# ingonyama-zk/icicle

Hardware: AMD Instinct MI355X
Metric: bn254_msm_2^26_per_sec (higher is better)
Workload: dtype u32x8 (254-bit integer field, 29-bit-limb Montgomery); 1 GPU; BN254 G1 MSM, 2^26 uniform scalars x 2^26 distinct affine bases per GPU, batch 1, inputs resident in HBM, precompute_factor 1

## Files before the change

icicle_amd/csrc/bigfield.hpp:

```cpp
#pragma once
#include <cstdint>
#include "field_consts.h"
#include "mont_asm.hpp"

#if defined(__HIPCC__)
  #include <hip/hip_runtime.h>
  #define HD __host__ __device__ __forceinline__
#else
  #define HD inline __attribute__((always_inline))
#endif

#ifdef BIGFIELD_BOUNDS
  #include <cassert>
  #include <cstdio>
  #define BF_BOUND_DECL                                                                                                \
    double bnd = 0;                                                                                                    \
    bool sg = false;                                                                                                   \
    double slo = 0, shi = 0, llo = 0, lhi = 0, tlo = 0, thi = 0;
  #define BF_SET_BOUND(x, v) ((x).bnd = (v), (x).sg = false)
  #define BF_ASSERT(cond, msg)                                                                                         \
    do {                                                                                                               \
      if (!(cond)) {                                                                                                   \
        fprintf(stderr, "bigfield bound violation: %s (%s:%d)\n", msg, __FILE__, __LINE__);                            \
        assert(false);                                                                                                 \
// ... 414 lines not shown
        r.l[i] = a.l[i] + b.l[i];
#ifdef BIGFIELD_BOUNDS
      const SB x = sview(a), y = sview(b);
      sset(r, SB{x.lo + y.lo, x.hi + y.hi, x.llo + y.llo, x.lhi + y.lhi, x.tlo + y.tlo, x.thi + y.thi});
#endif
      return r;
    }
    static HD fe ssub(const fe& a, const fe& b)
    {
      fe r;
#pragma unroll
      for (int i = 0; i < N; i++)
        r.l[i] = a.l[i] - b.l[i];
#ifdef BIGFIELD_BOUNDS
      const SB x = sview(a), y = sview(b);
      sset(r, SB{x.lo - y.hi, x.hi - y.lo, x.llo - y.lhi, x.lhi - y.llo, x.tlo - y.thi, x.thi - y.tlo});
#endif
      return r;
    }
    static HD fe sneg(const fe& a)
    {
      fe r;
#pragma unroll
      for (int i = 0; i < N; i++)
        r.l[i] = 0u - a.l[i];
#ifdef BIGFIELD_BOUNDS
      const SB x = sview(a);
      sset(r, SB{-x.hi, -x.lo, -x.lhi, -x.llo, -x.thi, -x.tlo});
#endif
      return r;
    }
    static HD fe sadd2(const fe& a, const fe& b)
    {
      fe r;
#pragma unroll
      for (int i = 0; i < N; i++)
        r.l[i] = (a.l[i] << 1) + b.l[i];
#ifdef BIGFIELD_BOUNDS
      const SB x = sview(a), y = sview(b);
      sset(r, SB{2 * x.lo + y.lo, 2 * x.hi + y.hi, 2 * x.llo + y.llo, 2 * x.lhi + y.lhi, 2 * x.tlo + y.tlo, 2 * x.thi + y.thi});
#endif
      return r;
    }
    static HD fe scneg(const fe& a, bool negate)
    {
      fe r;
      const uint32_t s = negate ? 0xffffffffu : 0u, o = negate ? 1u : 0u;
#pragma unroll
      for (int i = 0; i < N; i++)
        r.l[i] = (a.l[i] ^ s) + o;
#ifdef BIGFIELD_BOUNDS
      const SB x = sview(a);
      auto mn = [](double u, double v) { return u < v ? u : v; };
      auto mx = [](double u, double v) { return u > v ? u : v; };
      sset(r, SB{mn(x.lo, -x.hi), mx(x.hi, -x.lo), mn(x.llo, -x.lhi), mx(x.lhi, -x.llo), mn(x.tlo, -x.thi), mx(x.thi, -x.tlo)});
#endif
      return r;
    }
    static HD fe snormalise(const fe& a)
    {
      fe r;
      int32_t c = 0;
#pragma unroll
      for (int i = 0; i < N - 1; i++) {
        const int32_t t = (int32_t)a.l[i] + c;
        r.l[i] = (uint32_t)t & MASK;
        c = t >> RB;
      }
      r.l[N - 1] = a.l[N - 1] + (uint32_t)c;
#ifdef BIGFIELD_BOUNDS
      const SB x = sview(a);
      double clo = 0, chi = 0;
      for (int i = 0; i < N - 1; i++) {
        BF_ASSERT(x.llo + clo >= -I32_LIM && x.lhi + chi <= I32_LIM, "snormalise: limb + carry can leave int32");
        clo = __builtin_floor((x.llo + clo) / (double)(1u << RB));
        chi = __builtin_floor((x.lhi + chi) / (double)(1u << RB));
      }
      BF_ASSERT(x.tlo + clo >= -I32_LIM && x.thi + chi <= I32_LIM, "snormalise: top limb + carry can leave int32");
      sset(r, normalised(x.lo, x.hi));
#endif
      return r;
    }
    template <int K>
    static HD fe to_unsigned(const fe& a)
    {
      fe r;
      int32_t c = 0;
#pragma unroll
      for (int i = 0; i < N - 1; i++) {
        const int32_t t = (int32_t)(a.l[i] + kp<K>(i)) + c;
        r.l[i] = (uint32_t)t & MASK;
        c = t >> RB;
      }
      r.l[N - 1] = a.l[N - 1] + kp<K>(N - 1) + (uint32_t)c;
#ifdef BIGFIELD_BOUNDS
      const SB x = sview(a);
      BF_ASSERT(x.lo >= -(double)K, "to_unsigned: value can be below -K*p");
      BF_ASSERT(smag(x, 0) + (double)(1u << RB) + 8.0 <= I32_LIM && smag(x, N - 1) + (double)kp<K>(N - 1) + 8.0 <= I32_LIM, "to_unsigned: limb + K*p + carry can leave int32");
      BF_SET_BOUND(r, x.hi + (double)K);
      BF_ASSERT(r.bnd <= max_bound(), "to_unsigned result bound");
#endif
      return r;
    }

    template <bool TWO>
    static HD void sprod_generic(fe& r, const fe& a, const fe& b, const fe& c, const fe& d)
    {
      uint32_t m[N], o[N];
      int64_t acc = 0;
      auto term = [](uint32_t x, uint32_t y) { return (int64_t)(int32_t)x * (int64_t)(int32_t)y; };
#pragma unroll
      for (int k = 0; k < N; k++) {
#pragma unroll
        for (int i = 0; i <= k; i++) {
          acc += term(a.l[i], b.l[k - i]);
          if constexpr (TWO) acc += term(c.l[i], d.l[k - i]);
          if (i < k) acc += (int64_t)m[i] * (int64_t)PR::P[k - i];
        }
        m[k] = ((uint32_t)acc * PR::PINV) & MASK;
        acc += (int64_t)m[k] * (int64_t)PR::P[0];
        acc >>= RB;
      }
#pragma unroll
      for (int k = N; k < 2 * N - 1; k++) {
#pragma unroll
        for (int i = k - N + 1; i < N; i++) {
          acc += term(a.l[i], b.l[k - i]);
          if constexpr (TWO) acc += term(c.l[i], d.l[k - i]);
          acc += (int64_t)m[i] * (int64_t)PR::P[k - i];
        }
        o[k - N] = (uint32_t)acc & MASK;
        acc >>= RB;
      }
      o[N - 1] = (uint32_t)acc;
#pragma unroll
      for (int i = 0; i < N; i++)
        r.l[i] = o[i];
    }
    static HD fe smul(const fe& a, const fe& b)
    {
      fe r;
#ifdef BIGFIELD_BOUNDS
      sset_mul(r, a, b);
#endif
#if defined(__HIP_DEVICE_COMPILE__) && !defined(BIGFIELD_NO_ASM)
      if constexpr (N == 9) {
        mont_smul_asm9<PR>(r.l, a.l, b.l);
        return r;
      }
#endif
      sprod_generic<false>(r, a, b, a, b);
      return r;
    }
    static HD void smul_inplace(fe& a, const fe& b)
    {
#if defined(__HIP_DEVICE_COMPILE__) && !defined(BIGFIELD_NO_ASM)
      if constexpr (N == 9) {
        mont_smul_inplace_asm9<PR>(a.l, b.l);
        return;
      }
#endif
      a = smul(a, b);
    }
    static HD fe ssqr(const fe& a)
    {
      fe r;
// ... 197 lines not shown
```

icicle_amd/csrc/ec.hpp:

```cpp
#pragma once
#include "bigfield.hpp"
#include "fq2.hpp"
#include <type_traits>

#if defined(__HIPCC__)
  #define EC_NOINLINE __host__ __device__ __noinline__
#else
  #define EC_NOINLINE __attribute__((noinline))
#endif

namespace icicle_hip {

  template <class C>
  struct EC {
    using F = std::conditional_t<C::EXT_DEGREE == 2, Fq2Ops<typename C::fq>, FieldOps<typename C::fq>>;
    using fe = typename F::fe;
    static constexpr int N32 = F::N32;

    struct Aff {
      fe x, y;
    };
    struct XYZZ {
      fe x, y, zz, zzz;
    };
// ... 153 lines not shown
          return;
        }
      }
      fe PPP = F::smul(P, PP);
      fe Q = F::smul(acc.x, PP);
      fe t = F::sadd2(Q, PPP);
      fe X3 = F::snormalise(F::ssub(F::ssqr(R), t));
      fe d = F::ssub(Q, X3);
      acc.y = F::sneg(acc.y);
      F::smul_add_inplace_c(acc.y, R, d, PPP);
      F::smul_inplace(acc.zz, PP);
      F::smul_inplace(acc.zzz, PPP);
      acc.x = X3;
    }

    static HD Proj proj_identity()
    {
      Proj r;
      r.x = F::zero();
      r.y = F::one();
      r.z = F::zero();
      return r;
    }
    static HD Proj to_proj(const XYZZ& a, bool empty)
    {
      if (empty) return proj_identity();
      Proj r;
      if constexpr (SIGNED_MADD) {
        XYZZ s = a;
        F::sassume_normalised(s.x, -4.0, 6.0);
        F::sassume_normalised(s.y, -1.0, 4.0);
        F::sassume_normalised(s.zz, -0.25, 2.0);
        F::sassume_normalised(s.zzz, -0.25, 2.0);
        const fe zz1 = F::smul(s.zz, F::plain_one());
        r.x = F::template to_unsigned<1>(F::smul(s.x, s.zzz));
        r.y = F::template to_unsigned<1>(F::smul(s.y, s.zz));
        r.z = F::template to_unsigned<1>(F::smul(zz1, s.zzz));
      } else {
        const fe zz1 = F::mul_base(a.zz, F::base_plain_one());
        r.x = F::mul(a.x, a.zzz);
        r.y = F::mul(a.y, a.zz);
        r.z = F::mul(zz1, a.zzz);
      }
      return r;
    }
    static HD Proj to_proj(const Aff& a)
    {
      Proj r;
      r.x = a.x;
      r.y = a.y;
      r.z = F::one();
      return r;
    }
    static HD Proj add(const Proj& p, const Proj& q)
    {
      if constexpr (C::EXT_DEGREE == 2)
        return add_call(p, q);
      else
        return add_body(p, q);
    }
    static EC_NOINLINE Proj add_call(const Proj& p, const Proj& q) { return add_body(p, q); }
    static HD Proj add_body(const Proj& p, const Proj& q)
    {
      fe t0 = F::mul(p.x, q.x);
      fe t1 = F::mul(p.y, q.y);
      fe t2 = F::mul(p.z, q.z);
      fe t3 = F::mul(F::add(p.x, p.y), F::add(q.x, q.y));
      t3 = F::template sub<4>(t3, F::add(t0, t1));
      fe t4 = F::mul(F::add(p.y, p.z), F::add(q.y, q.z));
      t4 = F::template sub<4>(t4, F::add(t1, t2));
      fe t5 = F::mul(F::add(p.x, p.z), F::add(q.x, q.z));
      t5 = F::template sub<4>(t5, F::add(t0, t2));
      fe t0_3 = F::add(F::dbl(t0), t0);
      fe bt2 = F::mul(b3(), t2);
      fe z3 = F::add(t1, bt2);
      fe t1m = F::template sub<2>(t1, bt2);
      fe y3 = F::mul(b3(), t5);
      Proj r;
      r.x = F::template sub<2>(F::mul(t3, t1m), F::mul(t4, y3));
      r.y = F::add(F::mul(t1m, z3), F::mul(y3, t0_3));
      r.z = F::add(F::mul(z3, t4), F::mul(t0_3, t3));
      return r;
    }
    static HD Proj dbl(const Proj& p)
    {
      if constexpr (C::EXT_DEGREE == 2)
        return dbl_call(p);
      else
        return dbl_body(p);
    }
    static EC_NOINLINE Proj dbl_call(const Proj& p) { return dbl_body(p); }
    static HD Proj dbl_body(const Proj& p)
    {
      fe t0 = F::sqr(p.y);
      fe z8 = F::dbl(F::dbl(F::dbl(t0)));
      fe t1 = F::mul(p.y, p.z);
      fe t2 = F::mul(b3(), F::sqr(p.z));
      Proj r;
      fe x3 = F::mul(t2, z8);
      fe y3 = F::add(t0, t2);
      r.z = F::mul(t1, z8);
      fe t2_3 = F::add(F::dbl(t2), t2);
      fe t0m = F::template sub<4>(t0, t2_3);
      r.y = F::add(x3, F::mul(t0m, y3));
      r.x = F::dbl(F::mul(t0m, F::mul(p.x, p.y)));
      return r;
    }

    struct Jac {
      fe x, y, z;
    };
    static HD Jac to_jac(const Proj& p)
    {
      Jac r;
      fe zz = F::sqr(p.z);
      r.x = F::mul(p.x, p.z);
      r.y = F::mul(p.y, zz);
      r.z = p.z;
      return r;
    }
    static HD Proj from_jac(const Jac& j)
    {
      if (F::is_zero(j.z)) return proj_identity();
      Proj r;
      fe zz = F::sqr(j.z);
      r.x = F::mul(j.x, j.z);
      r.y = j.y;
      r.z = F::mul(zz, j.z);
      return r;
    }
    static HD Jac dbl_jac(const Jac& p)
    {
      fe A = F::sqr(p.x);
      fe B = F::sqr(p.y);
      fe CC = F::sqr(B);
      fe t = F::sqr(F::add(p.x, B));
      fe D = F::below4(F::dbl(F::template sub<4>(t, F::add(A, CC))));
      fe E = F::add(F::dbl(A), A);
      fe Fv = F::sqr(E);
      Jac r;
      r.x = F::below4(F::template sub<8>(Fv, F::dbl(D)));
      fe m = F::mul(E, F::template sub<4>(D, r.x));
      fe c8 = F::dbl(F::below4(F::dbl(F::dbl(CC))));
      r.y = F::below4(F::template sub<8>(m, c8));
      r.z = F::dbl(F::mul(p.y, p.z));
      return r;
    }

    static HD Jac dbl_jac_lazy(const Jac& p)
    {
      if constexpr (C::EXT_DEGREE == 2) {
        return dbl_jac(p);
      } else {
        fe A = F::sqr(p.x);
        fe B = F::sqr(p.y);
        fe CC = F::sqr(B);
        fe t = F::sqr(F::add(p.x, B));
        fe D = F::below4(F::dbl(F::template sub<4>(t, F::add(A, CC))));
        fe E = F::add(F::dbl(A), A);
        fe Fv = F::sqr(E);
        Jac r;
        r.x = F::template sub<8>(Fv, F::dbl(D));
        fe m = F::mul(E, F::template sub<16>(D, r.x));
        r.y = F::template sub<16>(m, F::dbl(F::dbl(F::dbl(CC))));
        r.z = F::dbl(F::mul(p.y, p.z));
        return r;
// ... 105 lines not shown
```

icicle_amd/csrc/msm_impl.hpp:

```cpp
#pragma once
#include "common.h"
#include "ec.hpp"
#include "ec_dbl_quad.hpp"
#include "msm_plan.h"
#include <algorithm>
#include <tuple>

namespace icicle_hip {

  template <class C>
  __global__ __launch_bounds__(256) void k_bases_stage(const uint32_t* __restrict__ in, uint32_t* __restrict__ out, size_t ncoord, bool in_refmont)
  {
    using BF = FieldOps<typename C::fq>;
    size_t t = blockIdx.x * (size_t)blockDim.x + threadIdx.x;
    if (t >= ncoord) return;
    uint32_t w[BF::N32];
#pragma unroll
    for (int i = 0; i < BF::N32; i++)
      w[i] = in[t * BF::N32 + i];
    if (in_refmont) {
      typename BF::fe cst;
#pragma unroll
      for (int k = 0; k < BF::N; k++)
        cst.l[k] = C::fq::REFMONT_TO_CANON[k];
// ... 733 lines not shown
    }
    const size_t wp = bucket / nb;
    bases += (wp / wpf) * bases_stride;
    const uint32_t total = count[bucket];
    const uint32_t cnt = min(total - min(total, start), seg);
    const uint32_t* src = sorted + wp * cap + offs[bucket] + start;
    typename E::XYZZ acc;
    bool empty = true;
    auto load4 = [&](uint32_t j) {
      uint4 v;
      __builtin_memcpy(&v, src + j, 16);
      return v;
    };
    uint4 cur = load4(0), nxt = cur;
    for (uint32_t j = 0; j < cnt; j++) {
      if ((j & 3u) == 0) nxt = load4(j + 4);
      const uint32_t e = cur.x;
      cur.x = cur.y, cur.y = cur.z, cur.z = cur.w;
      if ((j & 3u) == 3u) cur = nxt;
      const uint4* p = reinterpret_cast<const uint4*>(bases + (size_t)(e & 0x7fffffffu) * PW);
      uint32_t w[PW];
#pragma unroll
      for (int q = 0; q < PW / 4; q++) {
        const uint4 v = p[q];
        w[4 * q] = v.x;
        w[4 * q + 1] = v.y;
        w[4 * q + 2] = v.z;
        w[4 * q + 3] = v.w;
      }
      if (__builtin_expect(E::words_are_zero(w), 0)) continue;
      typename E::Aff a = E::cneg_madd(E::load_plain(w), (e >> 31) != 0);
      E::madd(acc, empty, a);
    }
    *dst = E::to_proj(acc, empty);
  }

  template <class C>
  __global__ __launch_bounds__(64) void k_fold_overflow(typename EC<C>::Proj* __restrict__ buckets, const typename EC<C>::Proj* __restrict__ ovf_part, const OvfSeg* __restrict__ ovf, const uint32_t* __restrict__ firsts, const uint32_t* __restrict__ ovf_count, uint32_t ovf_cap)
  {
    using E = EC<C>;
    __shared__ typename E::Proj sh[64];
    const uint32_t n = min(ovf_count[0], ovf_cap), nfirst = ovf_count[1];
    const uint32_t mx = ovf_count[2];
    const uint32_t G = mx <= 2 ? 1u : (mx <= 32 ? 4u : (mx <= 256 ? 16u : 64u)), per_block = 64 / G;
    const uint32_t lane = threadIdx.x, sub = lane / G, gl = lane % G;
    for (uint32_t q0 = blockIdx.x * per_block; q0 < nfirst; q0 += gridDim.x * per_block) {
      const uint32_t q = q0 + sub;
      const bool act = q < nfirst;
      const uint32_t o = act ? firsts[q] : 0;
      const uint32_t ne = act ? min(ovf[o].nextra, n - o) : 0;
      typename E::Proj v = E::proj_identity();
      for (uint32_t k = gl; k < ne; k += G)
        v = E::add(v, ovf_part[o + k]);
      sh[lane] = v;
      __syncthreads();
      for (uint32_t s = G / 2; s >= 1; s >>= 1) {
        if (gl < s) {
          v = E::add(v, sh[lane + s]);
          sh[lane] = v;
        }
        __syncthreads();
      }
      if (act && gl == 0) buckets[ovf[o].bucket] = E::add(buckets[ovf[o].bucket], v);
      __syncthreads();
    }
  }

  template <class C>
  struct ReduceWindowLanes {
    static constexpr int value = (sizeof(typename EC<C>::Proj) * 256 <= 60 * 1024) ? 256 : 128;
  };
  template <class P>
  __device__ __forceinline__ P proj_shfl_down(const P& v, int d)
  {
    static_assert(sizeof(P) % 4 == 0, "projective point is a whole number of words");
    P r;
    const uint32_t* src = reinterpret_cast<const uint32_t*>(&v);
    uint32_t* dst = reinterpret_cast<uint32_t*>(&r);
#pragma unroll
    for (size_t i = 0; i < sizeof(P) / 4; i++)
      dst[i] = __shfl_down(src[i], d);
    return r;
  }
  template <class C>
  __device__ __forceinline__ typename EC<C>::Proj wave_suffix_sum(typename EC<C>::Proj v, int lane)
  {
    using E = EC<C>;
    for (int d = 1; d < 64; d <<= 1) {
      const typename E::Proj o = proj_shfl_down(v, d);
      if (lane + d < 64) v = E::add(v, o);
    }
    return v;
  }
  template <class C>
  __device__ __forceinline__ typename EC<C>::Proj wave_sum(typename EC<C>::Proj v, int lane)
  {
    using E = EC<C>;
    for (int d = 32; d >= 1; d >>= 1) {
      const typename E::Proj o = proj_shfl_down(v, d);
      if (lane < d) v = E::add(v, o);
    }
    return v;
  }

  template <class C>
  __global__ __launch_bounds__(64) void k_reduce_wave(const typename EC<C>::Proj* __restrict__ buckets, typename EC<C>::Proj* __restrict__ chunkV, typename EC<C>::Proj* __restrict__ chunkT, typename EC<C>::Proj* __restrict__ winsum_direct, uint32_t nb_stride, uint32_t nb_wide, uint32_t m_wide, uint32_t seg_lo, uint32_t nsegr, uint32_t nlo_w, uint32_t nseg_lo, uint32_t m_lo)
  {
    using E = EC<C>;
    const int lane = threadIdx.x;
    const uint32_t nlo_blocks = nlo_w * nseg_lo;
    size_t wp;
    uint32_t ch, nb, lch;
    uint32_t m;
    if (blockIdx.x < nlo_blocks) {
      wp = blockIdx.x / nseg_lo, lch = blockIdx.x % nseg_lo, ch = lch, nb = nb_wide / 2, m = m_lo;
    } else {
      const uint32_t r = blockIdx.x - nlo_blocks;
      wp = nlo_w + r / nsegr, lch = r % nsegr, ch = seg_lo + lch, nb = nb_wide, m = m_wide;
    }
    const size_t oi = wp * nsegr + lch;
    const uint32_t k0 = ch * 64u * m;
    const typename E::Proj* b = buckets + wp * nb_stride;
    typename E::Proj line = E::proj_identity(), tri0 = E::proj_identity();
    for (int i = (int)m - 1; i >= 0; i--) {
      const uint32_t k = k0 + 64u * (uint32_t)i + (uint32_t)lane;
      tri0 = E::add(tri0, line);
      if (k < nb) line = E::add(line, b[k]);
    }
    const typename E::Proj suf = wave_suffix_sum<C>(line, lane);
    typename E::Proj x = proj_shfl_down(suf, 1);
    if (lane == 63) x = E::proj_identity();
    for (int q = 0; q < 6; q++)
      tri0 = E::dbl(tri0);
    const typename E::Proj v = wave_sum<C>(E::add(x, tri0), lane);
    if (lane == 0) {
      if (winsum_direct) {
        winsum_direct[oi] = E::add(v, suf);
      } else {
        chunkV[oi] = v;
        chunkT[oi] = suf;
      }
    }
  }

  template <class C>
  __global__ __launch_bounds__(64) void k_reduce_small(const typename EC<C>::Proj* __restrict__ buckets, typename EC<C>::Proj* __restrict__ winsum, uint32_t nb, uint32_t lw_log, uint32_t nwindows)
  {
    using E = EC<C>;
    const uint32_t lane = threadIdx.x, LW = 1u << lw_log, rows = nb >> lw_log;
    const uint32_t sl = lane & (LW - 1u);
    const size_t wp = (size_t)blockIdx.x * (64u >> lw_log) + (lane >> lw_log);
    const bool act = wp < nwindows;
    const typename E::Proj* b = buckets + (act ? wp : 0) * nb;
    typename E::Proj line = E::proj_identity(), tri0 = E::proj_identity();
    for (int i = (int)rows - 1; i >= 0; i--) {
      tri0 = E::add(tri0, line);
      if (act) line = E::add(line, b[(uint32_t)i * LW + sl]);
    }
    typename E::Proj suf = line;
    for (uint32_t d = 1; d < LW; d <<= 1) {
      const typename E::Proj o = proj_shfl_down(suf, (int)d);
      if (sl + d < LW) suf = E::add(suf, o);
    }
    typename E::Proj x = proj_shfl_down(suf, 1);
    if (sl == LW - 1u) x = E::proj_identity();
    for (uint32_t q = 0; q < lw_log; q++)
      tri0 = E::dbl(tri0);
    typename E::Proj v = E::add(x, tri0);
    for (uint32_t d = LW >> 1; d >= 1; d >>= 1) {
      const typename E::Proj o = proj_shfl_down(v, (int)d);
      if (sl < d) v = E::add(v, o);
    }
    if (act && sl == 0) winsum[wp] = E::add(v, suf);
  }

  template <class C>
  __global__ __launch_bounds__(ReduceWindowLanes<C>::value) void k_reduce_window(const typename EC<C>::Proj* __restrict__ chunkV, const typename EC<C>::Proj* __restrict__ chunkT, typename EC<C>::Proj* __restrict__ winsum, uint32_t nsegr_wide, uint32_t seg_lo_wide, uint32_t log_chunk_wide, uint32_t nlo_w, uint32_t nseg_lo, uint32_t log_chunk_lo)
  {
    const uint32_t nsegr = blockIdx.x < nlo_w ? nseg_lo : nsegr_wide, seg_lo = blockIdx.x < nlo_w ? 0u : seg_lo_wide;
    const uint32_t log_chunk = blockIdx.x < nlo_w ? log_chunk_lo : log_chunk_wide;
    using E = EC<C>;
    constexpr int RWL = ReduceWindowLanes<C>::value;
    __shared__ typename E::Proj sh[RWL];
    const int NW = blockDim.x / 64;
    const int wp = blockIdx.x, tid = threadIdx.x, lane = tid & 63, wave = tid >> 6;
    const bool have = (uint32_t)tid < nsegr;
    const typename E::Proj t = have ? chunkT[(size_t)wp * nsegr_wide + tid] : E::proj_identity();
    typename E::Proj u = have ? E::add(chunkV[(size_t)wp * nsegr_wide + tid], t) : E::proj_identity();
    const typename E::Proj suf = wave_suffix_sum<C>(t, lane);
    if (lane == 0) sh[wave] = suf;
    __syncthreads();
    typename E::Proj x = proj_shfl_down(suf, 1);
    if (lane == 63) x = E::proj_identity();
    typename E::Proj ttot = E::proj_identity();
    for (int w = NW - 1; w >= 0; w--) {
      if (w > wave) x = E::add(x, sh[w]);
      ttot = E::add(ttot, sh[w]);
    }
    __syncthreads();
    auto block_sum = [&](typename E::Proj v) {
      sh[tid] = v;
      __syncthreads();
      for (int s2 = blockDim.x / 2; s2 >= 1; s2 >>= 1) {
        if (tid < s2) {
          v = E::add(v, sh[tid + s2]);
          sh[tid] = v;
        }
        __syncthreads();
      }
      return v;
    };
    const typename E::Proj U = block_sum(u);
    typename E::Proj X = block_sum(x);
    if (tid == 0) {
      if (seg_lo) X = E::add(X, E::mul_small(ttot, seg_lo));
      for (uint32_t q = 0; q < log_chunk; q++)
        X = E::dbl(X);
      winsum[wp] = E::add(U, X);
    }
  }

  template <class C>
  __device__ __forceinline__ typename EC<C>::Proj reduce_quad_add(const typename EC<C>::Proj& a, const typename EC<C>::Proj& b, uint32_t role)
  {
    return EcQuadAdd<C>::add(a, b, role);
  }
  template <class C>
  __device__ __forceinline__ typename EC<C>::Proj reduce_quad_dbl(const typename EC<C>::Proj& a, uint32_t role)
  {
    if constexpr (has_small_b3<C>::value)
      return EcDblSmallB<C>::dbl_quad(a, role);
    else
      return EC<C>::dbl(a);
  }
  template <class C>
  __global__ __launch_bounds__(64) void k_reduce_wave_quad(const typename EC<C>::Proj* __restrict__ buckets, typename EC<C>::Proj* __restrict__ chunkV, typename EC<C>::Proj* __restrict__ chunkT, typename EC<C>::Proj* __restrict__ winsum_direct, uint32_t nb, uint32_t m, uint32_t nsegr)
  {
    using E = EC<C>;
    using Proj = typename E::Proj;
    const uint32_t role = threadIdx.x & 3u;
    const int lane = (int)(threadIdx.x >> 2);
    const size_t wp = blockIdx.x / nsegr;
    const uint32_t ch = blockIdx.x % nsegr;
    const uint32_t k0 = ch * 16u * m;
    const Proj* b = buckets + wp * nb;
    Proj line = E::proj_identity(), tri0 = E::proj_identity();
    for (int i = (int)m - 1; i >= 0; i--) {
      const uint32_t k = k0 + 16u * (uint32_t)i + (uint32_t)lane;
      tri0 = reduce_quad_add<C>(tri0, line, role);
      if (k < nb) line = reduce_quad_add<C>(line, b[k], role);
    }
    Proj suf = line;
    for (int d = 1; d < 16; d <<= 1) {
      const Proj o = proj_shfl_down(suf, 4 * d);
      if (lane + d < 16) suf = reduce_quad_add<C>(suf, o, role);
    }
    Proj x = proj_shfl_down(suf, 4);
    if (lane == 15) x = E::proj_identity();
    for (int q = 0; q < 4; q++)
      tri0 = reduce_quad_dbl<C>(tri0, role);
    Proj v = reduce_quad_add<C>(x, tri0, role);
    for (int d = 8; d >= 1; d >>= 1) {
      const Proj o = proj_shfl_down(v, 4 * d);
      if (lane < d) v = reduce_quad_add<C>(v, o, role);
    }
    if (lane == 0) {
      const size_t oi = wp * nsegr + ch;
      if (winsum_direct) {
        const Proj w = reduce_quad_add<C>(v, suf, role);
        if (role == 0) winsum_direct[oi] = w;
      } else if (role == 0) {
        chunkV[oi] = v;
        chunkT[oi] = suf;
      }
    }
  }
  template <class C>
  __global__ __launch_bounds__(256) void k_reduce_window_quad(const typename EC<C>::Proj* __restrict__ chunkV, const typename EC<C>::Proj* __restrict__ chunkT, typename EC<C>::Proj* __restrict__ winsum, uint32_t nsegr, uint32_t chunk)
  {
    using E = EC<C>;
    using Proj = typename E::Proj;
    __shared__ Proj sh[64];
    const int wp = blockIdx.x, tid = threadIdx.x;
    const uint32_t role = (uint32_t)tid & 3u;
    const int q = tid >> 2, lane = q & 15, wave = q >> 4;
    const int NQ = blockDim.x >> 2, NW = (blockDim.x + 63) / 64;
    const bool have = (uint32_t)q < nsegr;
    const Proj t = have ? chunkT[(size_t)wp * nsegr + q] : E::proj_identity();
    const Proj u = have ? reduce_quad_add<C>(chunkV[(size_t)wp * nsegr + q], t, role) : E::proj_identity();
    Proj suf = t;
    for (int d = 1; d < 16; d <<= 1) {
      const Proj o = proj_shfl_down(suf, 4 * d);
      if (lane + d < 16) suf = reduce_quad_add<C>(suf, o, role);
    }
    if (lane == 0 && role == 0) sh[wave] = suf;
    __syncthreads();
    Proj x = proj_shfl_down(suf, 4);
    if (lane == 15) x = E::proj_identity();
    for (int w = NW - 1; w > wave; w--)
      x = reduce_quad_add<C>(x, sh[w], role);
    __syncthreads();
// ... 615 lines not shown
        const uint32_t own_g = coresident ? 0u : own_max;
        k_b_plan<<<1, 1024, 0, sq>>>(offA, bstart, np_g, (int)tw, sp.hb, sp.nblk, p0, own_g);
        LAUNCH_CHECK("k_b_plan", sq);
        if (own_g) {
          k_b_owned<1024><<<np_g, 1024, ldsOwn, sq>>>(partA, offA, count, offs, sorted, (int)tw, pf, sp, cap, nb, p0, own_g);
          LAUNCH_CHECK("k_b_owned", sq);
        } else {
          HIP_TRY(hipMemsetAsync(count + bk0, 0, nbk_g * 4, sq), ICICLE_COPY_FAILED);
        }
        k_b_count<<<nblkB, 1024, ((size_t)1 << sp.lb) * 4, sq>>>(partA, offA, bstart, count, np_g, (int)tw, sp, cap, nb, p0);
        LAUNCH_CHECK("k_b_count", sq);
        if (own_g) {
          k_b_scan_part<<<np_g, 1024, 0, sq>>>(offA, count, offs, cursor, (int)tw, sp, nb, p0, own_g);
        } else {
          const uint32_t nch = (nb + SCAN_CHUNK - 1) / SCAN_CHUNK;
          k_scan_sums<<<dim3(nch, (unsigned)nw), 1024, 0, sq>>>(count + bk0, scan_g, nb);
          k_scan_apply<<<dim3(nch, (unsigned)nw), 1024, 0, sq>>>(count + bk0, scan_g, offs + bk0, cursor + bk0, nullptr, nb);
        }
        LAUNCH_CHECK("k_scan_buckets", sq);
        if (coresident) k_b_scatter<CO_TPB><<<nblkB, CO_TPB, ldsB_co, sq>>>(partA, offA, bstart, cursor, sorted, np_g, (int)tw, pf, sp, cap, nb, p0);
        else k_b_scatter<1024><<<nblkB, 1024, ldsB, sq>>>(partA, offA, bstart, cursor, sorted, np_g, (int)tw, pf, sp, cap, nb, p0);
        LAUNCH_CHECK("k_b_scatter", sq);
      }
      uint32_t* ovfcnt = ws->ovfcnt.template as<uint32_t>() + 4 * g;
      if (NG == 1) HIP_TRY(hipMemsetAsync(ovfcnt, 0, MsmWorkspace<C>::OVFCNT_GROUP_BYTES, sq), ICICLE_COPY_FAILED);
      k_plan_overflow<<<(unsigned)((nbk_g + 255) / 256), 256, 0, sq>>>(count, nbk_g, pl.seg, ovfcnt, ws->ovf.template as<OvfSeg>() + g_ovf_off[g], ws->firsts.template as<uint32_t>() + g_ovf_off[g] + g, g_ovf_cap[g], bk0);
      LAUNCH_CHECK("k_plan_overflow", sq);
      {
        const unsigned szblk = (unsigned)((nbk_g + SZ_CHUNK - 1) / SZ_CHUNK);
        const size_t sz0 = (bk0 / SZ_CHUNK + (size_t)(NG - 1 - g)) * SZ_BINS;
        const uint32_t m = szblk * SZ_BINS, nch = (m + SCAN_CHUNK - 1) / SCAN_CHUNK;
        uint32_t* sztab = ws->sztab.template as<uint32_t>() + sz0;
        uint32_t* szoff = ws->szoff.template as<uint32_t>() + sz0;
        k_bsize_count<<<szblk, 1024, 0, sq>>>(count, sztab, nbk_g, pl.seg, bk0, nb, (uint32_t)pl.n_lo);
        k_scan_sums<<<dim3(nch, 1), 1024, 0, sq>>>(sztab, scan_g, m);
        k_scan_apply<<<dim3(nch, 1), 1024, 0, sq>>>(sztab, scan_g, szoff, nullptr, nullptr, m);
        k_bsize_scatter<<<szblk, 1024, 0, sq>>>(count, szoff, ws->perm.template as<uint32_t>() + bk0, nbk_g, pl.seg, bk0, nb, (uint32_t)pl.n_lo);
        LAUNCH_CHECK("k_bsize_scatter", sq);
      }
      return ICICLE_SUCCESS;
    }

    icicle_error_t accumulate_group(int g, hipStream_t sq)
    {
      const int w0 = glo[g], nw = ghi[g] - glo[g];
      const size_t bk0 = (size_t)w0 * nb, nbk_g = (size_t)nw * nb;
      uint32_t* ovfcnt = ws->ovfcnt.template as<uint32_t>() + 4 * g;
      OvfSeg* ovf = ws->ovf.template as<OvfSeg>() + g_ovf_off[g];
      Proj* ovfpart = ws->ovfpart.template as<Proj>() + g_ovf_off[g];
      const uint32_t* firsts = ws->firsts.template as<uint32_t>() + g_ovf_off[g] + g;
      const uint32_t ocap = g_ovf_cap[g];
      KernelTimer::begin(0, sq);
      const int nlo_g = std::max(0, std::min(pl.n_lo, w0 + nw) - w0);
      const size_t nbk_used = nbk_g - (size_t)nlo_g * (nb / 2);
      const unsigned gridn = (unsigned)((nbk_used + ocap + 127) / 128);
      const size_t bstride = shared ? 0 : npts_one * PW;
      const MsmAccWaves aw = msm_acc_waves(sizeof(typename E::XYZZ) > 256, sizeof(typename E::XYZZ), E::F::N, co_ok, *kn);
      launch_accumulate<C>(aw, gridn, sq, acc_bases, sorted, count, offs, buckets, ovfpart, ovf, ovfcnt, ws->perm.template as<uint32_t>() + bk0, ocap, nb, nbk_used, cap, pl.seg, wpf, bstride);
      LAUNCH_CHECK("k_accumulate", sq);
      KernelTimer::end(0, sq);
      k_fold_overflow<C><<<std::min<uint32_t>(ocap, 4096), 64, 0, sq>>>(buckets, ovfpart, ovf, firsts, ovfcnt, ocap);
      LAUNCH_CHECK("k_fold_overflow", sq);
      return ICICLE_SUCCESS;
    }

    icicle_error_t reduce_group(int g, hipStream_t sq, uint32_t seg_lo, uint32_t nsegr)
    {
      const int w0 = glo[g], nw = ghi[g] - glo[g];
      const MsmReduceRoute rt = msm_reduce_route(nb, w0, nw, pl.n_lo, geo, seg_lo, nsegr, hook != nullptr, NG, bb, QUAD_OK, RWL, *kn);
      Proj* win = ws->win.template as<Proj>() + w0;
      Proj* cV = chunkV + (size_t)w0 * geo.nseg;
      Proj* cT = chunkT + (size_t)w0 * geo.nseg;
      const Proj* bk = buckets + (size_t)w0 * nb;
      switch (rt.chunk) {
      case MsmChunkKernel::wave_quad:
        if constexpr (QUAD_OK) k_reduce_wave_quad<C><<<(unsigned)((size_t)nw * rt.nsq), 64, 0, sq>>>(bk, cV, cT, rt.direct ? win : nullptr, nb, rt.mq, rt.nsq);
        LAUNCH_CHECK("k_reduce_wave_quad", sq);
        break;
      case MsmChunkKernel::small:
        k_reduce_small<C><<<(unsigned)(((size_t)nw + rt.per_wave - 1) / rt.per_wave), 64, 0, sq>>>(bk, win, nb, rt.lw_log, (uint32_t)nw);
        LAUNCH_CHECK("k_reduce_small", sq);
        break;
      case MsmChunkKernel::wave:
        k_reduce_wave<C><<<(unsigned)rt.nblocks, 64, 0, sq>>>(bk, cV, cT, rt.direct ? win : nullptr, nb, nb, geo.mrow, seg_lo, nsegr, rt.nlo_w, rt.nseg_lo, rt.mrow_lo);
        LAUNCH_CHECK("k_reduce_wave", sq);
        break;
      case MsmChunkKernel::none: break;
      }
      if (rt.window == MsmWindowKernel::window_quad) {
        if constexpr (QUAD_OK) k_reduce_window_quad<C><<<(unsigned)nw, rt.wthreads, 0, sq>>>(cV, cT, win, rt.wchunks, rt.wchunk_size);
        LAUNCH_CHECK("k_reduce_window_quad", sq);
      } else if (rt.window == MsmWindowKernel::window) {
        k_reduce_window<C><<<(unsigned)nw, rt.wthreads, 0, sq>>>(cV, cT, win, nsegr, seg_lo, geo.log_chunk, rt.nlo_w, rt.nseg_lo, rt.log_chunk_lo);
        LAUNCH_CHECK("k_reduce_window", sq);
      }
      if (NG > 1) {
        const int nbw = (nw + FINAL_WINDOWS_PER_BLOCK - 1) / FINAL_WINDOWS_PER_BLOCK;
        k_final<C><<<dim3((unsigned)nbw, 1), 64, 0, sq>>>(ws->win.template as<Proj>(), nullptr, wpf, ww, w0, nw, d_part.as<Proj>(), part_slot[g], 1);
        LAUNCH_CHECK("k_final(group)", sq);
      }
      return ICICLE_SUCCESS;
    }

    icicle_error_t host_combine()
    {
      Proj hw[64];
      HIP_TRY(hipMemcpyAsync(hw, ws->win.ptr(), (size_t)wpf * sizeof(Proj), hipMemcpyDeviceToHost, st), ICICLE_COPY_FAILED);
      KernelTimer::end(3, st);
      HIP_TRY(hipStreamSynchronize(st), ICICLE_SYNCHRONIZATION_FAILED);
      Proj acc = hw[wpf - 1];
      for (int w = wpf - 2; w >= 0; w--) {
        typename E::Jac j = E::to_jac(acc);
        for (int i = 0; i < pl.width(w); i++)
          j = E::dbl_jac(j);
        acc = E::add(E::from_jac(j), hw[w]);
      }
      if (cfg->are_results_on_device) {
        uint32_t words[RW];
        E::store_proj_canonical(words, acc);
        HIP_TRY(hipMemcpyAsync(results_v, words, sizeof(words), hipMemcpyHostToDevice, st), ICICLE_COPY_FAILED);
        HIP_TRY(hipStreamSynchronize(st), ICICLE_SYNCHRONIZATION_FAILED);
      } else {
        E::store_proj_canonical((uint32_t*)results_v, acc);
      }
      return ICICLE_SUCCESS;
    }

    icicle_error_t device_combine(MsmCombine how)
    {
      Proj* win = ws->win.template as<Proj>();
      uint32_t* res = d_res + (size_t)b0 * RW;
      if (how == MsmCombine::final_horner) {
        k_final_horner<C><<<(unsigned)((bb + 15) / 16), 64, 0, st>>>(win, res, wpf, ww, bb);
        LAUNCH_CHECK("k_final_horner", st);
        return ICICLE_SUCCESS;
      }
      const int nbw = (wpf + FINAL_WINDOWS_PER_BLOCK - 1) / FINAL_WINDOWS_PER_BLOCK;
      const bool partials = how == MsmCombine::final_then_combine;
      k_final<C><<<dim3((unsigned)nbw, (unsigned)bb), 64, 0, st>>>(win, res, wpf, ww, 0, wpf, partials ? d_part.as<Proj>() : nullptr, 0, bb);
      LAUNCH_CHECK("k_final", st);
      if (partials) {
        k_final_combine<C><<<(unsigned)((bb + 63) / 64), 64, 0, st>>>(d_part.as<Proj>(), res, nbw, bb);
        LAUNCH_CHECK("k_final_combine", st);
      }
      return ICICLE_SUCCESS;
    }

    icicle_error_t run_single_group(bool* result_written)
    {
      ICICLE_TRY(sort_group(0, st));
      KernelTimer::end(2, st);
      ICICLE_TRY(accumulate_group(0, st));
      KernelTimer::begin(3, st);
      uint32_t seg_lo = 0, nsegr = geo.nseg;
      if (hook) {
        bool skip = false;
        ICICLE_TRY(hook->after_accumulate(buckets, tw, nb, geo.nseg, geo.m, st, &skip, &seg_lo, &nsegr));
        if (skip) return ICICLE_SUCCESS;
      }
      ICICLE_TRY(reduce_group(0, st, seg_lo, nsegr));
      const MsmCombine how = msm_combine_route(cfg->are_results_on_device, cfg->is_async, batch, bb, hook != nullptr, wpf, *kn);
      if (how == MsmCombine::host) {
        *result_written = true;
        return host_combine();
      }
      ICICLE_TRY(device_combine(how));
      KernelTimer::end(3, st);
      return ICICLE_SUCCESS;
    }

    icicle_error_t run_pipelined()
    {
      hipEvent_t ev_sorted[MSM_MAX_GROUPS] = {nullptr}, ev_acc[MSM_MAX_GROUPS] = {nullptr};
      for (int g = 0; g < NG; g++) {
        ev_sorted[g] = ring_event();
        ev_acc[g] = ring_event();
// ... 217 lines not shown
```

icicle_amd/csrc/msm_plan.h:

```cpp
#pragma once
#include <algorithm>
#include <cstddef>
#include <cstdint>
#include <cstdlib>
#include "../../include/icicle_hip.h"

namespace icicle_hip {

  constexpr int MSM_MAX_GROUPS = 16;

  static inline int msm_window_groups(int tw, int want, int* glo, int* ghi)
  {
    int NG = std::max(1, std::min(std::min(want, MSM_MAX_GROUPS), tw / 2));
    if (tw < 4) NG = 1;
    const double unit = (double)tw / (NG <= 2 ? NG : NG - 1);
    double acc = 0;
    int hi = tw;
    for (int g = 0; g < NG; g++) {
      acc += (NG <= 2 || (g > 0 && g < NG - 1)) ? unit : unit / 2;
      int lo = g == NG - 1 ? 0 : std::max(0, tw - (int)(acc + 0.5));
      lo = std::min(lo, hi - 1);
      if (g < NG - 1) lo = std::max(lo, NG - 1 - g);
      glo[g] = lo, ghi[g] = hi;
      hi = lo;
// ... 39 lines not shown
      for (int cc = (small_c ? small_c : 2); cc <= (small_c ? small_c : 21); cc++) {
        const int w = (p.bits + 1 + cc - 1) / cc;
        const int wpf = (w + p.pf - 1) / p.pf;
        if (w > 1 && p.bits + 1 - cc * (w - 1) <= 3 && p.bits > 8) continue;
        if (!table && cfg.batch_size > 1 && n <= (1 << 17) && cc > 11) continue;
        const double nbk = (double)wpf * (double)(1u << (cc - 1));
        double cost;
        if (mid) {
          const double occupancy = std::max(1.0, 2.5 * 65536.0 / nbk);
          cost = (double)w * n * occupancy + ((table || n >= (1 << 22)) ? 4.0 : 2.0) * nbk;
        } else {
          cost = (double)w * n + 8.0 * nbk;
        }
        if (cost < best) {
          best = cost;
          c = cc;
        }
      }
    }
    c = std::min(22, std::max(2, c));
    p.c = c;
    p.nwin = (p.bits + 1 + c - 1) / c;
    p.wpf = (p.nwin + p.pf - 1) / p.pf;
    p.nb = 1u << (c - 1);
    if (cfg.c <= 0 && p.pf == 1 && p.bits == scalar_bits && std::max(1, cfg.batch_size) == 1 && (force_windows > 0 || (force_windows == 0 && n >= (1 << 23)))) {
      auto uniform_cost = [&](int w, double nbk) {
        const double occupancy = std::max(1.0, 2.5 * 65536.0 / nbk);
        return (double)w * n * occupancy + 4.0 * nbk;
      };
      int bestW = 0;
      double best = force_windows > 0 ? 1e300 : 0.995 * uniform_cost(p.nwin, (double)p.nwin * p.nb);
      for (int W = (force_windows > 0 ? force_windows : 2); W <= (force_windows > 0 ? force_windows : 40); W++) {
        const int clo = p.bits / W, x = p.bits - clo * W;
        if (x == 0 || clo + 1 > 22 || clo < (force_windows > 0 ? 2 : 12)) continue;
        const double nbk = (double)(W - x) * (double)(1u << (clo - 1)) + (double)x * (double)(1u << clo);
        const double cost = force_windows > 0 ? 0.0 : uniform_cost(W, nbk);
        if (cost < best) best = cost, bestW = W;
      }
      if (bestW > 0) {
        const int clo = p.bits / bestW, x = p.bits - clo * bestW;
        p.c = clo + 1;
        p.nwin = p.wpf = bestW;
        p.n_lo = bestW - x;
        p.negate = true;
        p.nb = 1u << (p.c - 1);
      }
    }
    {
      const double avg = (double)n * ((double)p.nwin / p.wpf) / (double)(p.n_lo > 0 ? p.nb / 2 : p.nb);
      uint32_t sgm = 64;
      while ((double)sgm < 2.0 * avg)
        sgm <<= 1;
      p.seg = sgm;
    }
    return p;
  }

  constexpr int SORT_EPT = 16;
  constexpr uint32_t SORT_TS = 1024 * SORT_EPT;
  constexpr uint32_t SCAN_CHUNK = 8192;
  constexpr uint32_t CHUNKB_LOG = 17;
  constexpr uint32_t PASSB_OWN_MAX_DEFAULT = 1u << 18;
  constexpr uint32_t SZ_BINS = 257;
  constexpr uint32_t SZ_CHUNK = 16384;
  constexpr int FINAL_WINDOWS_PER_BLOCK = 16;
#if defined(__HIPCC__)
  __host__ __device__
#endif
  static inline size_t tile_lds_bytes(uint32_t D, uint32_t TS = SORT_TS) { return ((size_t)2 * D + TS + TS / 2 + 32) * 4; }

  struct MsmKnobs {
    int windows = 0;
    bool hb_set = false;
    int hb = 0;
    bool mrow_set = false;
    int mrow = 0;
    int groups = MSM_DEFAULT_GROUPS;
    bool coresident = true;
    bool acc_waves_set = false;
    int acc_waves = 0;
    bool reduce_balance = false;
    bool reduce_small = true;
    bool reduce_quad = true;
    bool host_combine = true;
    bool batch_horner = true;
  };
  inline const MsmKnobs& msm_env_knobs()
  {
    static const MsmKnobs knobs = [] {
      MsmKnobs k;
      auto on_unless_0 = [](const char* name) { const char* e = getenv(name); return !(e && atoi(e) == 0); };
      if (const char* e = getenv("ICICLE_HIP_MSM_WINDOWS")) k.windows = atoi(e);
      if (const char* e = getenv("ICICLE_HIP_MSM_HB")) k.hb_set = true, k.hb = atoi(e);
      if (const char* e = getenv("ICICLE_HIP_MSM_MROW")) k.mrow_set = true, k.mrow = std::max(1, atoi(e));
      if (const char* e = getenv("ICICLE_HIP_MSM_GROUPS")) k.groups = atoi(e);
      k.coresident = on_unless_0("ICICLE_HIP_MSM_CORESIDENT");
      if (const char* e = getenv("ICICLE_HIP_MSM_ACC_WAVES")) k.acc_waves_set = true, k.acc_waves = atoi(e);
      if (const char* e = getenv("ICICLE_HIP_MSM_REDUCE_BALANCE")) k.reduce_balance = atoi(e) != 0;
      k.reduce_small = on_unless_0("ICICLE_HIP_MSM_REDUCE_SMALL");
      k.reduce_quad = on_unless_0("ICICLE_HIP_MSM_REDUCE_QUAD");
      k.host_combine = on_unless_0("ICICLE_HIP_MSM_HOST_COMBINE");
      k.batch_horner = on_unless_0("ICICLE_HIP_MSM_BATCH_HORNER");
      return k;
    }();
    return knobs;
  }

  struct SortPlan {
    int hb, lb;
    int jb;
    int chunk_log;
    int nblk;
  };
  static inline bool msm_sort_plan(int n, int c, int pf, const MsmKnobs& kn, SortPlan* sp)
  {
    const int kb = c - 1;
    int hb = kb <= 10 ? kb : (kb + 1) / 2;
    if (kn.hb_set) hb = kn.hb;
    hb = std::max(kb - 11, std::min(std::min(kb, 10), hb));
    if (hb < 0 || hb > 10 || kb - hb > 11) return false;
    sp->hb = hb;
    sp->lb = kb - hb;
    sp->jb = 0;
    while ((1 << sp->jb) < pf)
      sp->jb++;
    int logn = 0;
    while (((size_t)1 << logn) < (size_t)n)
      logn++;
    const int max_chunk = 31 - sp->lb - sp->jb;
    if (max_chunk < 10) return false;
    sp->chunk_log = std::max(10, std::min(max_chunk, std::max(17, logn - 9)));
    if (sp->chunk_log < logn - 9) return false;
    sp->nblk = (int)(((size_t)n + ((size_t)1 << sp->chunk_log) - 1) >> sp->chunk_log);
    return true;
  }

  struct MsmReduceGeom {
    uint32_t mrow;
    uint32_t m;
    uint32_t nseg;
    uint32_t log_chunk;
  };
  static inline MsmReduceGeom msm_reduce_geom(int batch, int wpf, uint32_t nb, uint32_t rwl, const MsmKnobs& kn)
  {
    uint32_t mrow_cap = 16;
    if (batch == 1 && nb >= 8192) {
      uint32_t need = (uint32_t)(((uint64_t)wpf * nb + 65535) / 65536), p2 = 2;
      while (p2 < need)
        p2 <<= 1;
      mrow_cap = std::min<uint32_t>(16, p2);
    }
    if (kn.mrow_set) mrow_cap = (uint32_t)kn.mrow;
    MsmReduceGeom g;
    g.mrow = std::max<uint32_t>(1, std::max<uint32_t>(nb / (64 * rwl), std::min<uint32_t>(mrow_cap, nb / 64)));
    g.m = 64 * g.mrow;
    g.nseg = std::max<uint32_t>(1, nb / g.m);
    g.log_chunk = 0;
    while ((1u << g.log_chunk) < g.m)
      g.log_chunk++;
    return g;
  }

  static inline int msm_batch_fold(const MsmPlan& pl, const SortPlan& sp, int n, size_t proj_bytes, size_t staged_base_bytes, size_t free_bytes, int batch, bool has_hook)
  {
    const size_t cap = (size_t)n * pl.pf;
    const size_t per_msm_bytes = (size_t)pl.nwin * n * 4 + (sp.lb == 0 ? 1 : 2) * (size_t)pl.wpf * cap * 4 + (size_t)pl.wpf * pl.nb * (proj_bytes + 12) +
                                 (size_t)pl.wpf * ((size_t)1 << sp.hb) * sp.nblk * 8 + staged_base_bytes;
    const size_t budget = std::min((size_t)48 << 30, free_bytes / 2);
    int BB = (int)std::max<size_t>(1, std::min<size_t>((size_t)batch, budget / std::max<size_t>(per_msm_bytes, 1)));
    BB = std::min(BB, std::max(1, 60000 / pl.wpf));
    if (has_hook && BB < batch) {
      BB = batch;
      if ((size_t)BB * pl.wpf > 60000) return 0;
    }
    return BB;
  }

  enum class MsmChunkKernel { none, wave_quad, small, wave };
  enum class MsmWindowKernel { none, window_quad, window };
  struct MsmReduceRoute {
    MsmChunkKernel chunk;
    MsmWindowKernel window;
    bool direct;
// ... 88 lines not shown
```

Measured before the change: 15.14 MSM/s.

## Use signed-limb projective addition in bucket reduction kernels

Adds a signed-limb complete projective addition (add_signed) that uses signed multiplies, fused mul-add pairs and small-constant multiplies for 3 and b3 in place of full field multiplications. The wave and window bucket-reduction kernels are templated to use it by default when the curve supports signed madd, converting back to unsigned form before doubling and before storing results. The aim is to lower the arithmetic cost of each reduction addition. In exchange it relies on bound assumptions about signed limbs and adds extra conversion steps and template instantiations.

New measurement: 15.40 MSM/s (median of 6 runs). +1.7%, better.

```diff
diff --git a/icicle_amd/csrc/bigfield.hpp b/icicle_amd/csrc/bigfield.hpp
--- a/icicle_amd/csrc/bigfield.hpp
+++ b/icicle_amd/csrc/bigfield.hpp
@@ -520,6 +520,32 @@
       return r;
     }
     template <int K>
+    static HD fe smul_small(const fe& a)
+    {
+      static_assert(K != 0 && K >= -64 && K <= 64, "a small constant");
+      fe r;
+      int64_t c = 0;
+#pragma unroll
+      for (int i = 0; i < N - 1; i++) {
+        const int64_t t = (int64_t)(int32_t)a.l[i] * K + c;
+        r.l[i] = (uint32_t)t & MASK;
+        c = t >> RB;
+      }
+      r.l[N - 1] = (uint32_t)((int64_t)(int32_t)a.l[N - 1] * K + c);
+#ifdef BIGFIELD_BOUNDS
+      const SB x = sview(a);
+      const double k = (double)K;
+      double clo = 0, chi = 0;
+      for (int i = 0; i < N - 1; i++) {
+        clo = __builtin_floor(((K > 0 ? x.llo : x.lhi) * k + clo) / (double)(1u << RB));
+        chi = __builtin_floor(((K > 0 ? x.lhi : x.llo) * k + chi) / (double)(1u << RB));
+      }
+      BF_ASSERT((K > 0 ? x.tlo : x.thi) * k + clo >= -I32_LIM && (K > 0 ? x.thi : x.tlo) * k + chi <= I32_LIM, "smul_small: top limb can leave int32");
+      sset(r, normalised(K > 0 ? k * x.lo : k * x.hi, K > 0 ? k * x.hi : k * x.lo));
+#endif
+      return r;
+    }
+    template <int K>
     static HD fe to_unsigned(const fe& a)
     {
       fe r;
diff --git a/icicle_amd/csrc/ec.hpp b/icicle_amd/csrc/ec.hpp
--- a/icicle_amd/csrc/ec.hpp
+++ b/icicle_amd/csrc/ec.hpp
@@ -259,6 +259,54 @@
       r.z = F::add(F::mul(z3, t4), F::mul(t0_3, t3));
       return r;
     }
+    static constexpr double ADD_LO = -1.5, ADD_HI = 1.75, ADD_IN_HI = 4.0;
+    static HD Proj add_signed(const Proj& p_, const Proj& q_)
+    {
+      static_assert(SIGNED_MADD, "add_signed: G1 over a 9-limb field");
+      Proj p = p_, q = q_;
+      F::sassume_normalised(p.x, ADD_LO, ADD_IN_HI);
+      F::sassume_normalised(p.y, ADD_LO, ADD_IN_HI);
+      F::sassume_normalised(p.z, ADD_LO, ADD_IN_HI);
+      F::sassume_normalised(q.x, ADD_LO, ADD_IN_HI);
+      F::sassume_normalised(q.y, ADD_LO, ADD_IN_HI);
+      F::sassume_normalised(q.z, ADD_LO, ADD_IN_HI);
+      const fe t0 = F::smul(p.x, q.x);
+      const fe t1 = F::smul(p.y, q.y);
+      const fe t2 = F::smul(p.z, q.z);
+      const fe m3 = F::smul(F::snormalise(F::sadd(p.x, p.y)), F::sadd(q.x, q.y));
+      const fe m4 = F::smul(F::snormalise(F::sadd(p.y, p.z)), F::sadd(q.y, q.z));
+      const fe m5 = F::smul(F::snormalise(F::sadd(p.x, p.z)), F::sadd(q.x, q.z));
+      const fe t3 = F::snormalise(F::ssub(m3, F::sadd(t0, t1)));
+      const fe t4 = F::snormalise(F::ssub(m4, F::sadd(t1, t2)));
+      const fe t5 = F::ssub(m5, F::sadd(t0, t2));
+      const fe t0_3 = F::template smul_small<3>(t0);
+      fe bt2, y3;
+      if constexpr (C::B3_SMALL != 0) {
+        bt2 = F::template smul_small<(int)C::B3_SMALL>(t2);
+        y3 = F::template smul_small<(int)C::B3_SMALL>(t5);
+      } else {
+        bt2 = F::smul(b3(), t2);
+        y3 = F::smul(b3(), t5);
+      }
+      const fe z3 = F::sadd(t1, bt2);
+      const fe t1m = F::ssub(t1, bt2);
+      Proj r;
+      r.x = F::smul_add(t3, t1m, F::sneg(t4), y3);
+      r.y = F::smul_add(t1m, z3, y3, t0_3);
+      r.z = F::smul_add(z3, t4, t0_3, t3);
+      F::sassume_normalised(r.x, ADD_LO, ADD_HI);
+      F::sassume_normalised(r.y, ADD_LO, ADD_HI);
+      F::sassume_normalised(r.z, ADD_LO, ADD_HI);
+      return r;
+    }
+    static HD Proj signed_to_unsigned(const Proj& p)
+    {
+      Proj r;
+      r.x = F::template to_unsigned<2>(p.x);
+      r.y = F::template to_unsigned<2>(p.y);
+      r.z = F::template to_unsigned<2>(p.z);
+      return r;
+    }
     static HD Proj dbl(const Proj& p)
     {
       if constexpr (C::EXT_DEGREE == 2)
diff --git a/icicle_amd/csrc/msm_impl.hpp b/icicle_amd/csrc/msm_impl.hpp
--- a/icicle_amd/csrc/msm_impl.hpp
+++ b/icicle_amd/csrc/msm_impl.hpp
@@ -839,28 +839,42 @@
       dst[i] = __shfl_down(src[i], d);
     return r;
   }
-  template <class C>
+  template <class C, bool SGN>
+  __device__ __forceinline__ typename EC<C>::Proj reduce_add(const typename EC<C>::Proj& a, const typename EC<C>::Proj& b)
+  {
+    if constexpr (SGN)
+      return EC<C>::add_signed(a, b);
+    else
+      return EC<C>::add(a, b);
+  }
+  template <class C, bool SGN>
+  __device__ __forceinline__ typename EC<C>::Proj reduce_unsigned(const typename EC<C>::Proj& a)
+  {
+    if constexpr (SGN)
+      return EC<C>::signed_to_unsigned(a);
+    else
+      return a;
+  }
+  template <class C, bool SGN = false>
   __device__ __forceinline__ typename EC<C>::Proj wave_suffix_sum(typename EC<C>::Proj v, int lane)
   {
-    using E = EC<C>;
     for (int d = 1; d < 64; d <<= 1) {
-      const typename E::Proj o = proj_shfl_down(v, d);
-      if (lane + d < 64) v = E::add(v, o);
+      const typename EC<C>::Proj o = proj_shfl_down(v, d);
+      if (lane + d < 64) v = reduce_add<C, SGN>(v, o);
     }
     return v;
   }
-  template <class C>
+  template <class C, bool SGN = false>
   __device__ __forceinline__ typename EC<C>::Proj wave_sum(typename EC<C>::Proj v, int lane)
   {
-    using E = EC<C>;
     for (int d = 32; d >= 1; d >>= 1) {
-      const typename E::Proj o = proj_shfl_down(v, d);
-      if (lane < d) v = E::add(v, o);
+      const typename EC<C>::Proj o = proj_shfl_down(v, d);
+      if (lane < d) v = reduce_add<C, SGN>(v, o);
     }
     return v;
   }
 
-  template <class C>
+  template <class C, bool SGN>
   __global__ __launch_bounds__(64) void k_reduce_wave(const typename EC<C>::Proj* __restrict__ buckets, typename EC<C>::Proj* __restrict__ chunkV, typename EC<C>::Proj* __restrict__ chunkT, typename EC<C>::Proj* __restrict__ winsum_direct, uint32_t nb_stride, uint32_t nb_wide, uint32_t m_wide, uint32_t seg_lo, uint32_t nsegr, uint32_t nlo_w, uint32_t nseg_lo, uint32_t m_lo)
   {
     using E = EC<C>;
@@ -881,21 +895,22 @@
     typename E::Proj line = E::proj_identity(), tri0 = E::proj_identity();
     for (int i = (int)m - 1; i >= 0; i--) {
       const uint32_t k = k0 + 64u * (uint32_t)i + (uint32_t)lane;
-      tri0 = E::add(tri0, line);
-      if (k < nb) line = E::add(line, b[k]);
-    }
-    const typename E::Proj suf = wave_suffix_sum<C>(line, lane);
+      tri0 = reduce_add<C, SGN>(tri0, line);
+      if (k < nb) line = reduce_add<C, SGN>(line, b[k]);
+    }
+    const typename E::Proj suf = wave_suffix_sum<C, SGN>(line, lane);
     typename E::Proj x = proj_shfl_down(suf, 1);
     if (lane == 63) x = E::proj_identity();
+    tri0 = reduce_unsigned<C, SGN>(tri0);
     for (int q = 0; q < 6; q++)
       tri0 = E::dbl(tri0);
-    const typename E::Proj v = wave_sum<C>(E::add(x, tri0), lane);
+    const typename E::Proj v = wave_sum<C, SGN>(reduce_add<C, SGN>(x, tri0), lane);
     if (lane == 0) {
       if (winsum_direct) {
-        winsum_direct[oi] = E::add(v, suf);
+        winsum_direct[oi] = reduce_unsigned<C, SGN>(reduce_add<C, SGN>(v, suf));
       } else {
-        chunkV[oi] = v;
-        chunkT[oi] = suf;
+        chunkV[oi] = reduce_unsigned<C, SGN>(v);
+        chunkT[oi] = reduce_unsigned<C, SGN>(suf);
       }
     }
   }
@@ -931,7 +946,7 @@
     if (act && sl == 0) winsum[wp] = E::add(v, suf);
   }
 
-  template <class C>
+  template <class C, bool SGN>
   __global__ __launch_bounds__(ReduceWindowLanes<C>::value) void k_reduce_window(const typename EC<C>::Proj* __restrict__ chunkV, const typename EC<C>::Proj* __restrict__ chunkT, typename EC<C>::Proj* __restrict__ winsum, uint32_t nsegr_wide, uint32_t seg_lo_wide, uint32_t log_chunk_wide, uint32_t nlo_w, uint32_t nseg_lo, uint32_t log_chunk_lo)
   {
     const uint32_t nsegr = blockIdx.x < nlo_w ? nseg_lo : nsegr_wide, seg_lo = blockIdx.x < nlo_w ? 0u : seg_lo_wide;
@@ -943,16 +958,16 @@
     const int wp = blockIdx.x, tid = threadIdx.x, lane = tid & 63, wave = tid >> 6;
     const bool have = (uint32_t)tid < nsegr;
     const typename E::Proj t = have ? chunkT[(size_t)wp * nsegr_wide + tid] : E::proj_identity();
-    typename E::Proj u = have ? E::add(chunkV[(size_t)wp * nsegr_wide + tid], t) : E::proj_identity();
-    const typename E::Proj suf = wave_suffix_sum<C>(t, lane);
+    typename E::Proj u = have ? reduce_add<C, SGN>(chunkV[(size_t)wp * nsegr_wide + tid], t) : E::proj_identity();
+    const typename E::Proj suf = wave_suffix_sum<C, SGN>(t, lane);
     if (lane == 0) sh[wave] = suf;
     __syncthreads();
     typename E::Proj x = proj_shfl_down(suf, 1);
     if (lane == 63) x = E::proj_identity();
     typename E::Proj ttot = E::proj_identity();
     for (int w = NW - 1; w >= 0; w--) {
-      if (w > wave) x = E::add(x, sh[w]);
-      ttot = E::add(ttot, sh[w]);
+      if (w > wave) x = reduce_add<C, SGN>(x, sh[w]);
+      ttot = reduce_add<C, SGN>(ttot, sh[w]);
     }
     __syncthreads();
     auto block_sum = [&](typename E::Proj v) {
@@ -960,7 +975,7 @@
       __syncthreads();
       for (int s2 = blockDim.x / 2; s2 >= 1; s2 >>= 1) {
         if (tid < s2) {
-          v = E::add(v, sh[tid + s2]);
+          v = reduce_add<C, SGN>(v, sh[tid + s2]);
           sh[tid] = v;
         }
         __syncthreads();
@@ -970,10 +985,11 @@
     const typename E::Proj U = block_sum(u);
     typename E::Proj X = block_sum(x);
     if (tid == 0) {
-      if (seg_lo) X = E::add(X, E::mul_small(ttot, seg_lo));
+      if (seg_lo) X = reduce_add<C, SGN>(X, E::mul_small(reduce_unsigned<C, SGN>(ttot), seg_lo));
+      X = reduce_unsigned<C, SGN>(X);
       for (uint32_t q = 0; q < log_chunk; q++)
         X = E::dbl(X);
-      winsum[wp] = E::add(U, X);
+      winsum[wp] = reduce_unsigned<C, SGN>(reduce_add<C, SGN>(U, X));
     }
   }
 
@@ -1755,7 +1771,11 @@
         LAUNCH_CHECK("k_reduce_small", sq);
         break;
       case MsmChunkKernel::wave:
-        k_reduce_wave<C><<<(unsigned)rt.nblocks, 64, 0, sq>>>(bk, cV, cT, rt.direct ? win : nullptr, nb, nb, geo.mrow, seg_lo, nsegr, rt.nlo_w, rt.nseg_lo, rt.mrow_lo);
+        if (E::SIGNED_MADD && kn->reduce_signed) {
+          if constexpr (E::SIGNED_MADD) k_reduce_wave<C, true><<<(unsigned)rt.nblocks, 64, 0, sq>>>(bk, cV, cT, rt.direct ? win : nullptr, nb, nb, geo.mrow, seg_lo, nsegr, rt.nlo_w, rt.nseg_lo, rt.mrow_lo);
+        } else {
+          k_reduce_wave<C, false><<<(unsigned)rt.nblocks, 64, 0, sq>>>(bk, cV, cT, rt.direct ? win : nullptr, nb, nb, geo.mrow, seg_lo, nsegr, rt.nlo_w, rt.nseg_lo, rt.mrow_lo);
+        }
         LAUNCH_CHECK("k_reduce_wave", sq);
         break;
       case MsmChunkKernel::none: break;
@@ -1764,7 +1784,11 @@
         if constexpr (QUAD_OK) k_reduce_window_quad<C><<<(unsigned)nw, rt.wthreads, 0, sq>>>(cV, cT, win, rt.wchunks, rt.wchunk_size);
         LAUNCH_CHECK("k_reduce_window_quad", sq);
       } else if (rt.window == MsmWindowKernel::window) {
-        k_reduce_window<C><<<(unsigned)nw, rt.wthreads, 0, sq>>>(cV, cT, win, nsegr, seg_lo, geo.log_chunk, rt.nlo_w, rt.nseg_lo, rt.log_chunk_lo);
+        if (E::SIGNED_MADD && kn->reduce_signed) {
+          if constexpr (E::SIGNED_MADD) k_reduce_window<C, true><<<(unsigned)nw, rt.wthreads, 0, sq>>>(cV, cT, win, nsegr, seg_lo, geo.log_chunk, rt.nlo_w, rt.nseg_lo, rt.log_chunk_lo);
+        } else {
+          k_reduce_window<C, false><<<(unsigned)nw, rt.wthreads, 0, sq>>>(cV, cT, win, nsegr, seg_lo, geo.log_chunk, rt.nlo_w, rt.nseg_lo, rt.log_chunk_lo);
+        }
         LAUNCH_CHECK("k_reduce_window", sq);
       }
       if (NG > 1) {
diff --git a/icicle_amd/csrc/msm_plan.h b/icicle_amd/csrc/msm_plan.h
--- a/icicle_amd/csrc/msm_plan.h
+++ b/icicle_amd/csrc/msm_plan.h
@@ -145,6 +145,7 @@
     bool reduce_balance = false;
     bool reduce_small = true;
     bool reduce_quad = true;
+    bool reduce_signed = true;
     bool host_combine = true;
     bool batch_horner = true;
   };
@@ -162,6 +163,7 @@
       if (const char* e = getenv("ICICLE_HIP_MSM_REDUCE_BALANCE")) k.reduce_balance = atoi(e) != 0;
       k.reduce_small = on_unless_0("ICICLE_HIP_MSM_REDUCE_SMALL");
       k.reduce_quad = on_unless_0("ICICLE_HIP_MSM_REDUCE_QUAD");
+      k.reduce_signed = on_unless_0("ICICLE_HIP_MSM_REDUCE_SIGNED");
       k.host_combine = on_unless_0("ICICLE_HIP_MSM_HOST_COMBINE");
       k.batch_horner = on_unless_0("ICICLE_HIP_MSM_BATCH_HORNER");
       return k;
```
